# pouryashirazian/FemBrain

Measured on AMD Instinct MI355X. Metric: FEM steps/sec (assemble+PCG) at 1M tets, higher is better.
Workload: dtype f64 arithmetic / f32 stored matrix

## Files before the change

### fembrain_amd/csrc/fem_persist.hip

```cpp
#include <cmath>
#include <cstring>

#include "fem_handle.h"
#include "pcg_pipe.hip.h"
#include "pcg_pipe2.hip.h"
#include "pcg_pipe_plan.h"

using namespace fb;

namespace fb {

struct PipeKernel {
  int rows;
  bool c16;
  int wmax, klt;
  bool timing, shard, bj, help, xyz;
  const void* fn;
};

namespace {

#define FB_PIPE1(C16, WMAX, KLT, TIMING, SHARD, BJ, HELP, XYZ) \
  {1, C16, WMAX, KLT, TIMING, SHARD, BJ, HELP, XYZ, (const void*)k_pcg_pipe<float, C16, WMAX, KLT, TIMING, SHARD, BJ, HELP, XYZ>}
#define FB_PIPE2(C16, SHARD, XYZ) {2, C16, 12, kPipe2Klt, false, SHARD, false, false, XYZ, (const void*)k_pcg_pipe2<C16, SHARD, XYZ>}
// ... 193 lines not shown
  FB_TRY(pipe_layout(h, kn, &want_xyz));
  ps.pipe_xyz = ps.pipe_rows == 2 && want_xyz;
  if (ps.pipe_rows != 1 || !(want_h || want_xyz) || w > kPipeMaxWaves) return FB_OK;
  const PipeTasks T = pipe_help_tasks(P.slice_off.data(), P.n_slices, ps.pipe_wg_first_host.empty() ? nullptr : ps.pipe_wg_first_host.data(), nb, w, h->c16 != 0, want_h,
                                      want_xyz, kn);
  if (!(T.all > 0 || T.deepest > 6 || want_xyz || kn.helpers == 2)) return FB_OK;
  FB_TRY(ps.pipe_tasks.upload(T.tasks, h->stream));
  ps.pipe_wmax = 12;
  ps.pipe_slots_dealt = T.deepest;
  ps.pipe_help_waves = T.help_waves; ps.pipe_n_help = T.most; ps.pipe_help_tasks = T.all;
  ps.pipe_xyz = want_xyz;
  if (kn.verbose) fprintf(stderr, "[fembrain] persistent solver: %d helper tasks (at most %d per workgroup), widest slice %d slots, mean %.1f, up to %d slots of a slice in LDS; a slot's gathers touch %.1f lines in planes, %.1f node by node -> %s\n", T.all, T.most, mx, mean, T.deepest, ps.pipe_gather_lines[0], ps.pipe_gather_lines[1], want_xyz ? "node by node" : "planes");
  return FB_OK;
}

int alloc_persist(fb_fem_s* h, int nb, const PersistKnobs& kn) {
  const FemPlan& P = h->plan;
  PersistState& ps = h->ps;
  hipStream_t s = h->stream;
  ZeroBatch zb(s);
  FB_TRY(ps.pipe_post.alloc((size_t)2 * nb * 4));
  zb.add(ps.pipe_post);
  ps.pipe_flag_extra = P.n_ranks > 1 ? kP2PMaxRanks : 0;
  FB_TRY(ps.pipe_flags.alloc((size_t)nb + ps.pipe_flag_extra + 16));
  zb.add(ps.pipe_flags);
  const size_t n_pad = (size_t)P.n_slices * 64, nv = (size_t)3 * P.n_local + 2;
  FB_TRY(ps.pipe_planes.alloc(2 * 3 * n_pad));
  zb.add(ps.pipe_planes);
  FB_TRY(ps.pipe_z.alloc(nv));
  FB_TRY(ps.pipe_s.alloc(nv));
  FB_TRY(ps.pipe_state.alloc(2));
  zb.add(ps.pipe_state);
  if (kn.timing) {
    FB_TRY(ps.persist_timing.alloc((size_t)nb * kPipeMaxWaves * 6));
    FB_TRY(ps.persist_timing.zero(s));
  } else {
    ps.persist_timing.release();
  }
  static_assert(kPipeMaxBlocks <= 256, "k_slice_producers holds 256 workgroups in its 8 mask words");
  FB_TRY(ps.pipe_owner.alloc((size_t)std::max(1, P.n_slices)));
  FB_TRY(ps.pipe_mask.alloc((size_t)std::max(1, P.n_slices) * 8));
  FB_TRY(ps.pipe_prod.alloc((size_t)nb * kPipeMaxProducers));
  FB_TRY(ps.pipe_prod_count.alloc((size_t)nb));
  FB_TRY(ps.pipe_prod_xcd.alloc((size_t)nb));
  FB_TRY(ps.pipe_stats.alloc(2));
  zb.add(ps.pipe_stats);
  FB_TRY(zb.flush());
  hipLaunchKernelGGL(k_slice_owner, dim3(ceil_div(nb, kBlock)), dim3(kBlock), 0, s, P.n_slices, nb, ps.pipe_wg_first.p, ps.pipe_owner.p);
  hipLaunchKernelGGL(k_slice_producers, dim3(ceil_div(std::max(1, P.n_slices), kWavesPerBlock)), dim3(kBlock), 0, s, P.n_slices, P.n_owned, h->slice_off.p, h->colidx.p,
                     ps.pipe_owner.p, ps.pipe_mask.p);
  hipLaunchKernelGGL(k_wg_producers, dim3(ceil_div(nb, kBlock)), dim3(kBlock), 0, s, P.n_slices, nb, ps.pipe_wg_first.p, ps.pipe_mask.p, kn.poll_all ? 1 : 0, ps.pipe_prod.p, ps.pipe_prod_count.p,
                     ps.pipe_prod_xcd.p, ps.pipe_stats.p);
  FB_HIP(hipGetLastError());
  ps.pipe_stats_pending = true;
  ps.pipe_max_producers = 0;
  FB_TRY(ps.pipe_xcc.alloc((size_t)nb));
  zb.add(ps.pipe_xcc);
  return zb.flush();
}

}

bool auto_matrix_f64(const fb_fem_s* h, int n_nodes, int n_ranks) {
  const int cus = h->cu_limit > 0 ? std::min(h->cu_limit, h->n_cu_device) : h->n_cu_device;
  const int nb = std::min(kPipeMaxBlocks, (cus / 8) * 8);
  const int w = nb >= 8 ? ceil_div(ceil_div(ceil_div(n_nodes, 64), 8), nb / 8) : 0;
  const bool shard_persist_asked = n_ranks > 1 && read_persist_knobs().sharded;
// ... 135 lines not shown
  pa.timeout_ticks = ps.persist_timeout_ticks;
  pa.timing = ps.persist_timing.p;
  pa.planes = ps.pipe_planes.p; pa.n_pad = ps.shard_persist ? (size_t)ceil_div(h->plan.n_local, 64) * 64 : (size_t)h->plan.n_slices * 64;
  pa.pstate = ps.pipe_state.p;
  pa.tasks = ps.pipe_tasks.p; pa.n_help = ps.pipe_n_help;
  pa.wg_first = ps.pipe_wg_first.p;
  pa.mirror = ps.pipe_mir.p; pa.mir_addr = ps.pipe_mir_addr.p; pa.mir_wg = ps.pipe_mir_wg.p; pa.mir_pool = ps.pipe_mir_pool.p;
  const int cwaves = K.rows == 2 ? ceil_div(ps.persist_waves, 2) : ps.persist_waves;
  pa.service = cwaves + ps.pipe_help_waves < ps.pipe_wmax ? 1 : 0;
  pa.prefetch_slots = ps.persist_waves >= 9 ? (K.rows == 2 ? 3 : 4) : 0;
  ShardArgs sa;
  memset(&sa, 0, sizeof sa);
  if (ps.shard_persist) {
    sa.rank = h->plan.rank; sa.n_ranks = h->plan.n_ranks; sa.n_owned = h->plan.n_owned; sa.n_halo = h->plan.n_local - h->plan.n_owned;
    sa.box = ps.sbox; sa.peer_box = ps.sbox_peers.p; sa.peer_seg = ps.sh_peer_seg.p; sa.halo_cap = ps.sbox_halo_cap;
    sa.halo_off = ps.sh_halo_off.p; sa.row_send_off = ps.sh_row_send_off.p; sa.row_send_rank = ps.sh_row_send_rank.p; sa.row_send_pos = ps.sh_row_send_pos.p;
    sa.wg_send_mask = ps.sh_wg_send_mask.p; sa.n_senders = ps.sh_n_senders.p; sa.proxy_wg = ps.sh_proxy_wg.p; sa.n_proxy = ps.sh_n_proxy; sa.wg_duty = ps.sh_wg_duty.p; sa.wg_range = ps.sh_wg_range.p;
    sa.delay_ticks = remote_delay_ticks();
  }
  SellView sv = sell_view(h);
  const float *vals = (const float*)h->vals.p, *dlo = (const float*)h->dlo.p;
  const double* inv = K.bj ? h->invblk.p : h->invdiag.p;
  void* args[] = {&sv, &vals, &dlo, &inv, &b, &h->x.p, &h->r.p, &h->Ad.p, &ps.pipe_z.p, &ps.pipe_s.p, &h->d.p, &h->st.p, &pa, &sa};
  const size_t lds = 160 * 1024;
  const dim3 grid(ps.persist_blocks), block(64 * (cwaves + ps.pipe_help_waves + pa.service));
  FB_HIP(hipEventRecord(h->ev_p[0], h->stream));
  FB_HIP(hipFuncSetAttribute(K.fn, hipFuncAttributeMaxDynamicSharedMemorySize, (int)lds));
  FB_HIP(hipLaunchKernel(K.fn, grid, block, args, lds, h->stream));
  FB_HIP(hipEventRecord(h->ev_p[1], h->stream));
  return FB_OK;
}

void print_pipe_timing(fb_fem_s* h) {
  std::vector<long long> tm((size_t)h->ps.persist_blocks * kPipeMaxWaves * 6);
  if (h->ps.persist_timing.download(tm.data(), tm.size(), h->stream) != FB_OK) return;
  (void)h->ps.persist_timing.zero(h->stream);
  const char* names[5] = {"publish (drained)", "flag+wait+acquire", "product", "sums sweep", "recurrences(+refresh)"};
  for (int k = 0; k < 5; k++) {
    double mn = 1e30, mx = 0, av = 0;
    int cnt = 0;
    for (int b = 0; b < h->ps.persist_blocks; b++)
      for (int w = 0; w < h->ps.persist_waves; w++) {
        const long long* t = &tm[((size_t)b * kPipeMaxWaves + w) * 6];
        if (t[5] <= 0) continue;
        const double us = (double)t[k] / (double)t[5] * 0.01;
        mn = std::min(mn, us); mx = std::max(mx, us); av += us; cnt++;
      }
    fprintf(stderr, "[fembrain] pipelined PCG %-22s per iteration: avg %.2f us  min %.2f  max %.2f (over %d waves)\n", names[k], av / std::max(cnt, 1), mn, mx, cnt);
  }
  if (h->ps.pipe_timing_level >= 2) {
    for (int k = 1; k <= 2; k++) {
      fprintf(stderr, "[fembrain] %s by wavefront:", names[k]);
      for (int w = 0; w < h->ps.persist_waves; w++) {
        double av = 0; int cnt = 0;
        for (int b = 0; b < h->ps.persist_blocks; b++) { const long long* t = &tm[((size_t)b * kPipeMaxWaves + w) * 6]; if (t[5] > 0) { av += (double)t[k] / (double)t[5] * 0.01; cnt++; } }
        fprintf(stderr, " %.2f", av / std::max(cnt, 1));
      }
      fprintf(stderr, "\n[fembrain] %s by XCD (avg / max over its workgroups' slowest wavefront):", names[k]);
      for (int x = 0; x < 8; x++) {
        double av = 0, mx = 0; int cnt = 0;
        for (int b = x; b < h->ps.persist_blocks; b += 8) {
          double wmx = 0;
          for (int w = 0; w < h->ps.persist_waves; w++) { const long long* t = &tm[((size_t)b * kPipeMaxWaves + w) * 6]; if (t[5] > 0) wmx = std::max(wmx, (double)t[k] / (double)t[5] * 0.01); }
          av += wmx; mx = std::max(mx, wmx); cnt++;
        }
        fprintf(stderr, " %.2f/%.2f", av / std::max(cnt, 1), mx);
      }
      fprintf(stderr, "\n");
    }
    std::vector<std::pair<double, int>> slow;
    for (int b = 0; b < h->ps.persist_blocks; b++) {
      double wmx = 0;
      for (int w = 0; w < h->ps.persist_waves; w++) { const long long* t = &tm[((size_t)b * kPipeMaxWaves + w) * 6]; if (t[5] > 0) wmx = std::max(wmx, (double)t[2] / (double)t[5] * 0.01); }
      slow.push_back({wmx, b});
    }
    std::sort(slow.begin(), slow.end());
    fprintf(stderr, "[fembrain] slowest product of a workgroup: median %.2f us, fastest", slow[slow.size() / 2].first);
    for (int k = 0; k < 6 && k < (int)slow.size(); k++) fprintf(stderr, " wg%d %.2f", slow[k].second, slow[k].first);
    fprintf(stderr, "; slowest");
    for (int k = 0; k < 12 && k < (int)slow.size(); k++) fprintf(stderr, " wg%d %.2f", slow[slow.size() - 1 - k].second, slow[slow.size() - 1 - k].first);
    fprintf(stderr, "\n");
  }
}

}

extern "C" {

int fb_fem_sharded_persist(fb_fem_t h) {
  if (!h) return 0;
  return h->ps.shard_persist && h->ps.persist ? 1 : 0;
}

int fb_fem_set_sharded_persist(fb_fem_t h, int on) {
  CHECK_HANDLE(h);
  if (!h->ps.shard_persist || !h->ps.sbox) return fail(FB_EINVAL, "the sharded persistent solver is not attached to this handle (FEMBRAIN_SHARDED_PERSIST=1 at creation, <= %d slices per CU)", 2 * (kPipeMaxWaves - 1));
  if (on && h->ps.persist_broken) return fail(FB_EDEVICE, "the sharded persistent solver of this handle timed out before; it stays with the two-launch iteration");
  FB_HIP(hipStreamSynchronize(h->stream));
  h->ps.persist = on != 0;
  return FB_OK;
}

int fb_fem_persist_info(fb_fem_t h, int* waves_per_cu, int* workgroups, int* lds_slots) {
  if (!h) return fail(FB_EINVAL, "null FEM handle");
  if (waves_per_cu) *waves_per_cu = h->ps.persist ? h->ps.persist_waves : 0;
  if (workgroups) *workgroups = h->ps.persist ? h->ps.persist_blocks : 0;
// ... 91 lines not shown
```

### fembrain_amd/csrc/pcg_pipe.hip.h

```cpp
#pragma once
#include "fem_kernels.h"
#include "pcg_pipe_stream.hip.h"
#include "pcg_pipe_mirror.h"

namespace fb {

constexpr int kPipeMaxWaves = 12;
constexpr int kPipeMaxBlocks = 256;
constexpr int kPipeSyncDoubles = 2 * 16 + 2 * kPipeMaxBlocks + 8;
constexpr int kPipeMaxProducers = 64;
constexpr int pipe_slot_bytes(bool c16) { return c16 ? 9 * 256 + 128 : 10 * 256; }
constexpr int pipe_lds_slots(bool c16) { return c16 ? 65 : 62; }
static_assert(sizeof(double) * kPipeSyncDoubles + (size_t)pipe_lds_slots(false) * pipe_slot_bytes(false) <= 160 * 1024, "LDS budget of k_pcg_pipe");
static_assert(sizeof(double) * kPipeSyncDoubles + (size_t)pipe_lds_slots(true) * pipe_slot_bytes(true) <= 160 * 1024, "LDS budget of k_pcg_pipe<c16>");
static_assert(mir_slot_bytes(true) == pipe_slot_bytes(true) && mir_slot_bytes(false) == pipe_slot_bytes(false) && mir_lds_slots(true) == pipe_lds_slots(true) &&
              mir_lds_slots(false) == pipe_lds_slots(false) && kMirWaves == kPipeMaxWaves, "the LDS window's planner sees the kernel's LDS");
static_assert(pipe_lds_slots(true) * pipe_slot_bytes(true) / 4 < 65536 && pipe_lds_slots(false) * pipe_slot_bytes(false) / 4 < 65536, "16-bit LDS word addresses of the mirror layers");

struct PipeArgs {
  unsigned long long* post;
  unsigned int* flags;
  unsigned int* error;
  unsigned int* seqs;
  const int* producers;
  const int* prod_count;
  const int* prod_xcd;
  int plain_local;
  unsigned int* xcc;
  int prefetch_slots;
  int service;
  int start;
  int n_iters;
  double eps2;
  int max_iter;
  long long timeout_ticks;
  long long* timing;
  double* planes;
  size_t n_pad;
  double* pstate;
  const int* wg_first;
  const int4* tasks;
  int n_help;
  const int4* mirror;
  const unsigned short* mir_addr;
  const int2* mir_wg;
  const int* mir_pool;
};
constexpr int kPipeTaskStride = 16;
constexpr int kPipeMaxHelpers = 8;
constexpr int pipe_help_slots(bool c16) { return c16 ? 6 : 5; }
static_assert(pipe_help_slots(true) * pipe_slot_bytes(true) >= kPipeMaxHelpers * 3 * 64 * 8 && pipe_help_slots(false) * pipe_slot_bytes(false) >= kPipeMaxHelpers * 3 * 64 * 8, "helpers' hand-over area");

__device__ __forceinline__ void st_sc1_u64(unsigned long long* p, unsigned long long v) { __hip_atomic_store(p, v, __ATOMIC_RELAXED, __HIP_MEMORY_SCOPE_AGENT); }
__device__ __forceinline__ void st_sc1_u32(unsigned int* p, unsigned int v) { __hip_atomic_store(p, v, __ATOMIC_RELAXED, __HIP_MEMORY_SCOPE_AGENT); }
__device__ __forceinline__ unsigned int ld_sc1_u32(const unsigned int* p) { return __hip_atomic_load(p, __ATOMIC_RELAXED, __HIP_MEMORY_SCOPE_AGENT); }
__device__ __forceinline__ void st_sc1_f64(double* p, double v) { __hip_atomic_store(p, v, __ATOMIC_RELAXED, __HIP_MEMORY_SCOPE_AGENT); }
__device__ __forceinline__ void st_sc1_xyz(double* p, double x, double y, double z) {
  typedef double d2 __attribute__((ext_vector_type(2)));
  const d2 xy = {x, y};
  asm volatile("global_store_dwordx4 %0, %1, off sc1\n\tglobal_store_dwordx2 %0, %2, off offset:16 sc1" : : "v"(p), "v"(xy), "v"(z) : "memory");
}
__device__ __forceinline__ uint4 ld_sc1_u128(const void* p) {
  uint4 v;
  asm volatile("global_load_dwordx4 %0, %1, off sc1\n\ts_waitcnt vmcnt(0)" : "=v"(v) : "v"(p) : "memory");
  return v;
}

__device__ __forceinline__ double uniform_f64(double v) {
  const long long b = __double_as_longlong(v);
  const unsigned int lo = __builtin_amdgcn_readfirstlane((unsigned int)(b & 0xffffffffLL)), hi = __builtin_amdgcn_readfirstlane((unsigned int)((unsigned long long)b >> 32));
  return __longlong_as_double((long long)(((unsigned long long)hi << 32) | lo));
}
__device__ __forceinline__ bool uniform_flag(bool f) { return __builtin_amdgcn_readfirstlane(f ? 1 : 0) != 0; }

__host__ __device__ inline void pipe_slices(int n_slices, int n_blocks, int b, int* first, int* count) {
  const int xcd = b & 7, j = b >> 3, per = n_blocks >> 3;
  const int chunk = (n_slices + 7) >> 3;
  const int lo = xcd * chunk;
  int len = n_slices - lo;
  len = len < 0 ? 0 : (len > chunk ? chunk : len);
  const int base = len / per, rem = len - base * per;
// ... 316 lines not shown
      const int2 pw = pa.mir_wg[blockIdx.x];
      unsigned int* lmat = (unsigned int*)(lds + kPipeSyncDoubles);
      for (int e = threadIdx.x; e < pw.y; e += blockDim.x) {
        const MT* src = vals + pa.mir_pool[(size_t)blockIdx.x * kMirPoolMax + e];
        unsigned int* pe = lmat + pw.x + (e >> 6) * 9 * 64 + (e & 63);
#pragma unroll
        for (int j = 0; j < 9; j++) pe[(3 * (j % 3) + j / 3) * 64] = __float_as_uint((float)src[j * 64]);
      }
    }
  }
  double* ypart = (double*)((char*)(lds + kPipeSyncDoubles) + (size_t)(pipe_lds_slots(C16) - pipe_help_slots(C16)) * pipe_slot_bytes(C16));
  int own_k1 = width, help_sl = -1, hk0 = 0, hk1 = 0, help_idx = 0, help_so = 0;
  unsigned int help_mask = 0u;
  if constexpr (HELP) {
    const int4 tk = pa.tasks[(size_t)blockIdx.x * kPipeTaskStride + wv];
    const bool helper = !live && !spare && tk.x >= 0;
    own_k1 = __builtin_amdgcn_readfirstlane(live ? tk.z : width);
    help_mask = (unsigned int)__builtin_amdgcn_readfirstlane(live ? tk.w : 0);
    help_sl = __builtin_amdgcn_readfirstlane(helper ? first + tk.x : -1);
    hk0 = __builtin_amdgcn_readfirstlane(helper ? tk.y : 0); hk1 = __builtin_amdgcn_readfirstlane(helper ? tk.z : 0);
    help_idx = __builtin_amdgcn_readfirstlane(helper ? tk.w : 0);
    help_so = __builtin_amdgcn_readfirstlane(sv.slice_off[help_sl < 0 ? 0 : help_sl]);
  }
  const int n_prod = pa.prod_count[blockIdx.x];
  int my_prod = -1;
  if (wv == 0 && n_prod >= 0 && lane < n_prod) my_prod = pa.producers[(size_t)blockIdx.x * kPipeMaxProducers + lane];

  unsigned int send_mask = 0u;
  ShardBoxLayout BL = {};
  if constexpr (SHARD) { send_mask = sa.wg_send_mask[blockIdx.x]; BL = shard_box_layout(sa.halo_cap); }
  unsigned int pub = pa.seqs[0], sums = pa.seqs[1];
  const long long t_limit = pa.timeout_ticks;
  bool failed = false;
  long long tm[TIMING ? 6 : 1] = {0}, tprev = TIMING ? wall_clock64() : 0;
  auto lap = [&](int k) { if (TIMING) { const long long t = wall_clock64(); tm[k] += t - tprev; tprev = t; } };

  const bool plain_cand = !SHARD && pa.plain_local != 0 && pa.prod_xcd[blockIdx.x] == 0;
  bool through = true, xcc_known = false;
  unsigned int my_xcc = 0u;
  if constexpr (!SHARD) {
    asm volatile("s_getreg_b32 %0, hwreg(HW_REG_XCC_ID, 0, 4)" : "=s"(my_xcc));
    if (threadIdx.x == 0) st_sc1_u32(pa.xcc + blockIdx.x, ((pub + 1u) << 4) | my_xcc);
  }
  static_assert(!XYZ || HELP, "the node-by-node vector comes with the table-driven instantiation");
  const size_t xs = XYZ ? 1 : pa.n_pad, cs = XYZ ? 3 : 1;
  auto publish = [&](const double* vin) {
    pub++;
    double* pl = pa.planes + (size_t)(pub & 1u) * 3 * pa.n_pad;
    if (rvalid) {
      if (XYZ && through) {
        st_sc1_xyz(pl + 3 * (size_t)row, vin[0], vin[1], vin[2]);
      } else if (through) {
#pragma unroll
        for (int a = 0; a < 3; a++) st_sc1_f64(pl + a * xs + cs * (size_t)row, vin[a]);
      } else {
#pragma unroll
        for (int a = 0; a < 3; a++) pl[a * xs + cs * (size_t)row] = vin[a];
      }
      if constexpr (SHARD) shard_send_row(sa, BL, pub, send_beg, send_end, vin);
    }
  };
  auto product = [&](const double* vin, double* y, bool post_sums, bool late_acquire) {
    double* pl = pa.planes + (size_t)(pub & 1u) * 3 * pa.n_pad;
    asm volatile("s_waitcnt vmcnt(0)" ::: "memory");
    __syncthreads();
    lap(0);
    if (post_sums) sums++;
// ... 34 lines not shown
            if (b < nb) {
              const uint4 f = ld_sc1_u128(pa.flags + b);
              ok = (int)(f.x - pub) >= 0 && (b + 1 >= nb || (int)(f.y - pub) >= 0) && (b + 2 >= nb || (int)(f.z - pub) >= 0) && (b + 3 >= nb || (int)(f.w - pub) >= 0);
            }
            if (__ballot(!ok) == 0ULL) break;
            if (ld_sc1_u32(pa.error) != 0u || wall_clock64() - t0 > t_limit) { failed = true; break; }
            __builtin_amdgcn_s_sleep(1);
          }
        }
      }
      if (failed && lane == 0) st_sc1_u32(pa.error, 1u);
      if (late_acquire) __builtin_amdgcn_fence(__ATOMIC_ACQUIRE, "agent");
      if (plain_cand && !xcc_known && !failed) {
        const bool same = my_prod < 0 || ld_sc1_u32(pa.xcc + my_prod) == ((pub << 4) | my_xcc);
        const bool all_same = __ballot(!same) == 0ULL;
        if (lane == 0) bc[5] = all_same ? 1.0 : 0.0;
      }
      asm volatile("s_waitcnt vmcnt(0)" ::: "memory");
      if (lane == 0) bc[3] = (failed || ld_sc1_u32(pa.error) != 0u) ? 1.0 : 0.0;
    }
    __syncthreads();
    lap(1);
    if (uniform_flag(bc[3] != 0.0 || (SHARD && bc[4] != 0.0))) { failed = true; return; }
    if (plain_cand && !xcc_known) { through = !uniform_flag(bc[5] != 0.0); xcc_known = true; }
    double y0 = 0, y1 = 0, y2 = 0;
    if (rvalid) {
      MT u00 = m00, u01 = m01, u02 = m02, u11 = m11, u12 = m12, u22 = m22;
      asm volatile("" : "+v"(u00), "+v"(u01), "+v"(u02), "+v"(u11), "+v"(u12), "+v"(u22));
      const double l00 = (double)u00, l01 = (double)u01, l02 = (double)u02, l11 = (double)u11, l12 = (double)u12, l22 = (double)u22;
      y0 = l00 * vin[0] + l01 * vin[1] + l02 * vin[2];
      y1 = l01 * vin[0] + l11 * vin[1] + l12 * vin[2];
      y2 = l02 * vin[0] + l12 * vin[1] + l22 * vin[2];
    }
    if (live) {
      if constexpr (kMir) {
        if (mir_a > 0) {
          int so_k = so;
          asm volatile("" : "+s"(so_k));
          pipe_stream_slots<C16, XYZ>(mir_a, ((unsigned int)so_k * 9u * 64u + (unsigned int)lane) * (unsigned int)sizeof(float),
                                      ((unsigned int)so_k * 64u + (unsigned int)lane) * (unsigned int)(C16 ? sizeof(short) : sizeof(int)), vals,
                                      C16 ? (const void*)sv.coldelta : (const void*)sv.colidx, pl, pl + xs, pl + 2 * xs, row, y0, y1, y2);
        }
        const unsigned int* lmt = (const unsigned int*)((const char*)(lds + kPipeSyncDoubles) + mir_tab) + lane;
        const unsigned int* lmat = (const unsigned int*)(lds + kPipeSyncDoubles);
#pragma unroll
        for (int k = 0; k < kMirMax; k++) if (k < mir_m) {
          unsigned int addr, col;
          if constexpr (C16) { const unsigned int wd = lmt[k * 64]; addr = wd >> 16; col = (unsigned int)(row + (int)(short)(wd & 0xffffu)); }
          else { col = lmt[k * 96]; addr = ((const unsigned short*)(lmt - lane + k * 96 + 64))[lane]; }
          const unsigned int* pk = lmat + addr;
          const double* xp = pl + cs * (size_t)col;
          const double x0 = xp[0], x1 = xp[xs], x2 = xp[2 * xs];
          y0 += (double)__uint_as_float(pk[0 * 64]) * x0 + (double)__uint_as_float(pk[3 * 64]) * x1 + (double)__uint_as_float(pk[6 * 64]) * x2;
          y1 += (double)__uint_as_float(pk[1 * 64]) * x0 + (double)__uint_as_float(pk[4 * 64]) * x1 + (double)__uint_as_float(pk[7 * 64]) * x2;
          y2 += (double)__uint_as_float(pk[2 * 64]) * x0 + (double)__uint_as_float(pk[5 * 64]) * x1 + (double)__uint_as_float(pk[8 * 64]) * x2;
        }
      }
      if (sizeof(MT) == 4 && KLT >= 16) {
        double gx[KLT][3];
#pragma unroll
        for (int k = 0; k < KLT; k++) {
          const unsigned int col = k < KL ? lds_col(k) : 0u;
          const double* xp = pl + cs * (size_t)col;
          gx[k][0] = k < KL ? xp[0] : 0.0; gx[k][1] = k < KL ? xp[xs] : 0.0; gx[k][2] = k < KL ? xp[2 * xs] : 0.0;
        }
#pragma unroll
        for (int k = 0; k < KLT; k++) if (k < KL) {
          const unsigned int* lk = lres + (size_t)k * kValWords * 64;
          const double x0 = gx[k][0], x1 = gx[k][1], x2 = gx[k][2];
          y0 += (double)__uint_as_float(lk[0 * 64]) * x0 + (double)__uint_as_float(lk[1 * 64]) * x1 + (double)__uint_as_float(lk[2 * 64]) * x2;
          y1 += (double)__uint_as_float(lk[3 * 64]) * x0 + (double)__uint_as_float(lk[4 * 64]) * x1 + (double)__uint_as_float(lk[5 * 64]) * x2;
          y2 += (double)__uint_as_float(lk[6 * 64]) * x0 + (double)__uint_as_float(lk[7 * 64]) * x1 + (double)__uint_as_float(lk[8 * 64]) * x2;
        }
      } else if (sizeof(MT) == 4) {
#pragma unroll
        for (int k = 0; k < KLT; k++) if (k < KL) {
          const unsigned int* lk = lres + (size_t)k * kValWords * 64;
          const double* xp = pl + cs * (size_t)lds_col(k);
          const double x0 = xp[0], x1 = xp[xs], x2 = xp[2 * xs];
          y0 += (double)__uint_as_float(lk[0 * 64]) * x0 + (double)__uint_as_float(lk[1 * 64]) * x1 + (double)__uint_as_float(lk[2 * 64]) * x2;
          y1 += (double)__uint_as_float(lk[3 * 64]) * x0 + (double)__uint_as_float(lk[4 * 64]) * x1 + (double)__uint_as_float(lk[5 * 64]) * x2;
          y2 += (double)__uint_as_float(lk[6 * 64]) * x0 + (double)__uint_as_float(lk[7 * 64]) * x1 + (double)__uint_as_float(lk[8 * 64]) * x2;
        }
        if constexpr (HELP) {
          for (int kb = KLT; kb < KL; kb += KLT) {
            double gx[KLT][3];
#pragma unroll
            for (int j = 0; j < KLT; j++) {
              const int k = min(kb + j, KL - 1);
              const double* xp = pl + cs * (size_t)lds_col(k);
              gx[j][0] = xp[0]; gx[j][1] = xp[xs]; gx[j][2] = xp[2 * xs];
            }
#pragma unroll
            for (int j = 0; j < KLT; j++) if (kb + j < KL) {
              const unsigned int* lk = lres + (size_t)(kb + j) * kValWords * 64;
              const double x0 = gx[j][0], x1 = gx[j][1], x2 = gx[j][2];
              y0 += (double)__uint_as_float(lk[0 * 64]) * x0 + (double)__uint_as_float(lk[1 * 64]) * x1 + (double)__uint_as_float(lk[2 * 64]) * x2;
              y1 += (double)__uint_as_float(lk[3 * 64]) * x0 + (double)__uint_as_float(lk[4 * 64]) * x1 + (double)__uint_as_float(lk[5 * 64]) * x2;
              y2 += (double)__uint_as_float(lk[6 * 64]) * x0 + (double)__uint_as_float(lk[7 * 64]) * x1 + (double)__uint_as_float(lk[8 * 64]) * x2;
            }
          }
        }
      }
      const int n_str = own_k1 - k_after;
      if (n_str > 0) {
        int so_k = so + k_after;
        asm volatile("" : "+s"(so_k));
        pipe_stream_slots<C16, XYZ>(n_str, ((unsigned int)so_k * 9u * 64u + (unsigned int)lane) * (unsigned int)sizeof(float),
                               ((unsigned int)so_k * 64u + (unsigned int)lane) * (unsigned int)(C16 ? sizeof(short) : sizeof(int)), vals,
                               C16 ? (const void*)sv.coldelta : (const void*)sv.colidx, pl, pl + xs, pl + 2 * xs, row, y0, y1, y2);
      }
    }
    if constexpr (HELP) if (help_sl >= 0) {
      double h0 = 0, h1 = 0, h2 = 0;
      int so_k = help_so + hk0;
      asm volatile("" : "+s"(so_k));
      if (hk1 > hk0)
      pipe_stream_slots<C16, XYZ>(hk1 - hk0, ((unsigned int)so_k * 9u * 64u + (unsigned int)lane) * (unsigned int)sizeof(float),
                             ((unsigned int)so_k * 64u + (unsigned int)lane) * (unsigned int)(C16 ? sizeof(short) : sizeof(int)), vals,
                             C16 ? (const void*)sv.coldelta : (const void*)sv.colidx, pl, pl + xs, pl + 2 * xs, help_sl * 64 + lane, h0, h1, h2);
      double* hp = ypart + (size_t)help_idx * 3 * 64 + lane;
      hp[0] = h0; hp[64] = h1; hp[128] = h2;
    }
    y[0] = y0; y[1] = y1; y[2] = y2;
    lap(2);
  };
  auto add_helpers = [&](double* y) {
    unsigned int m = help_mask;
    while (m) {
      const int hi = __ffs((int)m) - 1;
      m &= m - 1u;
      const double* hp = ypart + (size_t)hi * 3 * 64 + lane;
      y[0] += hp[0]; y[1] += hp[64]; y[2] += hp[128];
    }
  };
// ... 153 lines not shown
#pragma unroll
    for (int a = 0; a < 3; a++) {
      zr[a] = y[a] + beta * zr[a];
      sr[a] = wr[a] + beta * sr[a];
    }
    if (!refresh) {
      double m[3];
#pragma unroll
      for (int a = 0; a < 3; a++) wr[a] = wr[a] - alpha * zr[a];
      precond(wr, m);
      publish(m);
      published = true;
    }
    if constexpr (BJ) {
      double ur[3];
      precond(rr, ur);
#pragma unroll
      for (int a = 0; a < 3; a++) pr[a] = ur[a] + beta * pr[a];
    } else {
#pragma unroll
      for (int a = 0; a < 3; a++) pr[a] = iv[a] * rr[a] + beta * pr[a];
    }
#pragma unroll
    for (int a = 0; a < 3; a++) xr[a] = xr[a] + alpha * pr[a];
    if (refresh) {
      phase = PH_REFRESH_X;
    } else {
#pragma unroll
      for (int a = 0; a < 3; a++) rr[a] = rr[a] - alpha * sr[a];
    }
    lap(4);
  }
  if (TIMING && lane == 0) {
    for (int k = 0; k < 5; k++) atomicAdd((unsigned long long*)pa.timing + ((size_t)blockIdx.x * kPipeMaxWaves + wv) * 6 + k, (unsigned long long)tm[k]);
    atomicAdd((unsigned long long*)pa.timing + ((size_t)blockIdx.x * kPipeMaxWaves + wv) * 6 + 5, (unsigned long long)it_done);
  }
  if (failed) return;
  const bool capped = done && gamma > eps2 * rho0;
  if (rvalid) {
    unsigned int dof = 3u * (unsigned int)row;
    asm volatile("" : "+v"(dof));
    if (capped) {
#pragma unroll
      for (int a = 0; a < 3; a++) pg[dof + a] = xr[a];
    } else {
#pragma unroll
      for (int a = 0; a < 3; a++) xg[dof + a] = xr[a];
      if (!done) {
#pragma unroll
        for (int a = 0; a < 3; a++) { rg[dof + a] = rr[a]; wg[dof + a] = wr[a]; zg[dof + a] = zr[a]; sg[dof + a] = sr[a]; pg[dof + a] = pr[a]; }
      }
    }
  }
  if (blockIdx.x == 0 && threadIdx.x == 0) {
    st->rho0 = rho0; st->eps2 = eps2; st->max_iter = max_iter;
    st->iter = iter;
    st->rho[iter & 1] = done ? gamma : gamma_old;
    st->done = done ? 1 : 0;
    pa.pstate[0] = gamma_old; pa.pstate[1] = alpha_old;
    pa.seqs[0] = (SHARD && published) ? pub - 1u : pub; pa.seqs[1] = sums;
  }
}

}
```

Baseline: 64.26.

## Software-pipeline on-chip mirrored and resident SpMV slots in hand-written assembly

Replaces the compiler-generated loop over LDS-mirrored slots, and the separate loop over LDS-resident plain slots, with one inline-assembly loop. It keeps up to four slot gathers of x in flight and uses graded vmcnt waits, so the gather latency overlaps with the f64 multiply-adds of earlier slots. It also adds timing seams that split the product phase into streamed and on-chip parts, with matching host-side reporting. The hand-written asm hardcodes VGPR numbers and LDS offsets, which adds register pressure and correctness risk.

```diff
diff --git a/fembrain_amd/csrc/fem_persist.hip b/fembrain_amd/csrc/fem_persist.hip
--- a/fembrain_amd/csrc/fem_persist.hip
+++ b/fembrain_amd/csrc/fem_persist.hip
@@ -249,7 +249,7 @@
   FB_TRY(ps.pipe_state.alloc(2));
   zb.add(ps.pipe_state);
   if (kn.timing) {
-    FB_TRY(ps.persist_timing.alloc((size_t)nb * kPipeMaxWaves * 6));
+    FB_TRY(ps.persist_timing.alloc((size_t)nb * kPipeMaxWaves * kPipeTimingSlots));
     FB_TRY(ps.persist_timing.zero(s));
   } else {
     ps.persist_timing.release();
@@ -451,7 +451,7 @@
 }
 
 void print_pipe_timing(fb_fem_s* h) {
-  std::vector<long long> tm((size_t)h->ps.persist_blocks * kPipeMaxWaves * 6);
+  std::vector<long long> tm((size_t)h->ps.persist_blocks * kPipeMaxWaves * kPipeTimingSlots);
   if (h->ps.persist_timing.download(tm.data(), tm.size(), h->stream) != FB_OK) return;
   (void)h->ps.persist_timing.zero(h->stream);
   const char* names[5] = {"publish (drained)", "flag+wait+acquire", "product", "sums sweep", "recurrences(+refresh)"};
@@ -460,19 +460,39 @@
     int cnt = 0;
     for (int b = 0; b < h->ps.persist_blocks; b++)
       for (int w = 0; w < h->ps.persist_waves; w++) {
-        const long long* t = &tm[((size_t)b * kPipeMaxWaves + w) * 6];
+        const long long* t = &tm[((size_t)b * kPipeMaxWaves + w) * kPipeTimingSlots];
         if (t[5] <= 0) continue;
         const double us = (double)t[k] / (double)t[5] * 0.01;
         mn = std::min(mn, us); mx = std::max(mx, us); av += us; cnt++;
       }
     fprintf(stderr, "[fembrain] pipelined PCG %-22s per iteration: avg %.2f us  min %.2f  max %.2f (over %d waves)\n", names[k], av / std::max(cnt, 1), mn, mx, cnt);
   }
+  if (h->ps.kernel && h->ps.kernel->wmax == 12 && !h->ps.kernel->help) {
+    const char* parts[3] = {"product: streamed [0,a)", "product: on-chip run", "product: streamed rest"};
+    for (int k = 0; k < 3; k++) {
+      double av = 0, mx = 0, sav = 0;
+      int cnt = 0, wgs = 0;
+      for (int b = 0; b < h->ps.persist_blocks; b++) {
+        double slowest = -1, part = 0;
+        for (int w = 0; w < h->ps.persist_waves; w++) {
+          const long long* t = &tm[((size_t)b * kPipeMaxWaves + w) * kPipeTimingSlots];
+          if (t[5] <= 0) continue;
+          const double us = (double)(k == 0 ? t[6] : (k == 1 ? t[7] : t[2] - t[6] - t[7])) / (double)t[5] * 0.01;
+          av += us; mx = std::max(mx, us); cnt++;
+          if ((double)t[2] > slowest) { slowest = (double)t[2]; part = us; }
+        }
+        if (slowest >= 0) { sav += part; wgs++; }
+      }
+      fprintf(stderr, "[fembrain] pipelined PCG %-24s per iteration: avg %.2f us  max %.2f; in the slowest wavefront of a workgroup: avg %.2f\n", parts[k], av / std::max(cnt, 1), mx,
+              sav / std::max(wgs, 1));
+    }
+  }
   if (h->ps.pipe_timing_level >= 2) {
     for (int k = 1; k <= 2; k++) {
       fprintf(stderr, "[fembrain] %s by wavefront:", names[k]);
       for (int w = 0; w < h->ps.persist_waves; w++) {
         double av = 0; int cnt = 0;
-        for (int b = 0; b < h->ps.persist_blocks; b++) { const long long* t = &tm[((size_t)b * kPipeMaxWaves + w) * 6]; if (t[5] > 0) { av += (double)t[k] / (double)t[5] * 0.01; cnt++; } }
+        for (int b = 0; b < h->ps.persist_blocks; b++) { const long long* t = &tm[((size_t)b * kPipeMaxWaves + w) * kPipeTimingSlots]; if (t[5] > 0) { av += (double)t[k] / (double)t[5] * 0.01; cnt++; } }
         fprintf(stderr, " %.2f", av / std::max(cnt, 1));
       }
       fprintf(stderr, "\n[fembrain] %s by XCD (avg / max over its workgroups' slowest wavefront):", names[k]);
@@ -480,7 +500,7 @@
         double av = 0, mx = 0; int cnt = 0;
         for (int b = x; b < h->ps.persist_blocks; b += 8) {
           double wmx = 0;
-          for (int w = 0; w < h->ps.persist_waves; w++) { const long long* t = &tm[((size_t)b * kPipeMaxWaves + w) * 6]; if (t[5] > 0) wmx = std::max(wmx, (double)t[k] / (double)t[5] * 0.01); }
+          for (int w = 0; w < h->ps.persist_waves; w++) { const long long* t = &tm[((size_t)b * kPipeMaxWaves + w) * kPipeTimingSlots]; if (t[5] > 0) wmx = std::max(wmx, (double)t[k] / (double)t[5] * 0.01); }
           av += wmx; mx = std::max(mx, wmx); cnt++;
         }
         fprintf(stderr, " %.2f/%.2f", av / std::max(cnt, 1), mx);
@@ -490,7 +510,7 @@
     std::vector<std::pair<double, int>> slow;
     for (int b = 0; b < h->ps.persist_blocks; b++) {
       double wmx = 0;
-      for (int w = 0; w < h->ps.persist_waves; w++) { const long long* t = &tm[((size_t)b * kPipeMaxWaves + w) * 6]; if (t[5] > 0) wmx = std::max(wmx, (double)t[2] / (double)t[5] * 0.01); }
+      for (int w = 0; w < h->ps.persist_waves; w++) { const long long* t = &tm[((size_t)b * kPipeMaxWaves + w) * kPipeTimingSlots]; if (t[5] > 0) wmx = std::max(wmx, (double)t[2] / (double)t[5] * 0.01); }
       slow.push_back({wmx, b});
     }
     std::sort(slow.begin(), slow.end());
diff --git a/fembrain_amd/csrc/pcg_pipe.hip.h b/fembrain_amd/csrc/pcg_pipe.hip.h
--- a/fembrain_amd/csrc/pcg_pipe.hip.h
+++ b/fembrain_amd/csrc/pcg_pipe.hip.h
@@ -1,6 +1,7 @@
 #pragma once
 #include "fem_kernels.h"
 #include "pcg_pipe_stream.hip.h"
+#include "pcg_pipe_onchip.hip.h"
 #include "pcg_pipe_mirror.h"
 
 namespace fb {
@@ -47,6 +48,7 @@
   const int* mir_pool;
 };
 constexpr int kPipeTaskStride = 16;
+constexpr int kPipeTimingSlots = 8;
 constexpr int kPipeMaxHelpers = 8;
 constexpr int pipe_help_slots(bool c16) { return c16 ? 6 : 5; }
 static_assert(pipe_help_slots(true) * pipe_slot_bytes(true) >= kPipeMaxHelpers * 3 * 64 * 8 && pipe_help_slots(false) * pipe_slot_bytes(false) >= kPipeMaxHelpers * 3 * 64 * 8, "helpers' hand-over area");
@@ -429,7 +431,8 @@
   unsigned int pub = pa.seqs[0], sums = pa.seqs[1];
   const long long t_limit = pa.timeout_ticks;
   bool failed = false;
-  long long tm[TIMING ? 6 : 1] = {0}, tprev = TIMING ? wall_clock64() : 0;
+  long long tm[TIMING ? 7 : 1] = {0}, tprev = TIMING ? wall_clock64() : 0;
+  auto seam = [&](int k, long long& t) { if (TIMING) { const long long u = wall_clock64(); tm[k] += u - t; t = u; } };
   auto lap = [&](int k) { if (TIMING) { const long long t = wall_clock64(); tm[k] += t - tprev; tprev = t; } };
 
   const bool plain_cand = !SHARD && pa.plain_local != 0 && pa.prod_xcd[blockIdx.x] == 0;
@@ -530,6 +533,7 @@
       y1 = l01 * vin[0] + l11 * vin[1] + l12 * vin[2];
       y2 = l02 * vin[0] + l12 * vin[1] + l22 * vin[2];
     }
+    long long tseam = tprev;
     if (live) {
       if constexpr (kMir) {
         if (mir_a > 0) {
@@ -539,20 +543,10 @@
                                       ((unsigned int)so_k * 64u + (unsigned int)lane) * (unsigned int)(C16 ? sizeof(short) : sizeof(int)), vals,
                                       C16 ? (const void*)sv.coldelta : (const void*)sv.colidx, pl, pl + xs, pl + 2 * xs, row, y0, y1, y2);
         }
-        const unsigned int* lmt = (const unsigned int*)((const char*)(lds + kPipeSyncDoubles) + mir_tab) + lane;
-        const unsigned int* lmat = (const unsigned int*)(lds + kPipeSyncDoubles);
-#pragma unroll
-        for (int k = 0; k < kMirMax; k++) if (k < mir_m) {
-          unsigned int addr, col;
-          if constexpr (C16) { const unsigned int wd = lmt[k * 64]; addr = wd >> 16; col = (unsigned int)(row + (int)(short)(wd & 0xffffu)); }
-          else { col = lmt[k * 96]; addr = ((const unsigned short*)(lmt - lane + k * 96 + 64))[lane]; }
-          const unsigned int* pk = lmat + addr;
-          const double* xp = pl + cs * (size_t)col;
-          const double x0 = xp[0], x1 = xp[xs], x2 = xp[2 * xs];
-          y0 += (double)__uint_as_float(pk[0 * 64]) * x0 + (double)__uint_as_float(pk[3 * 64]) * x1 + (double)__uint_as_float(pk[6 * 64]) * x2;
-          y1 += (double)__uint_as_float(pk[1 * 64]) * x0 + (double)__uint_as_float(pk[4 * 64]) * x1 + (double)__uint_as_float(pk[7 * 64]) * x2;
-          y2 += (double)__uint_as_float(pk[2 * 64]) * x0 + (double)__uint_as_float(pk[5 * 64]) * x1 + (double)__uint_as_float(pk[8 * 64]) * x2;
-        }
+        seam(5, tseam);
+        const char* lbase = (const char*)(lds + kPipeSyncDoubles);
+        pipe_onchip_slots<C16>(mir_m, max(KL, 0), (const unsigned int*)(lbase + mir_tab) + lane, (const unsigned short*)(lbase + mir_tab) + lane, lres, lcd, lbase, pl, pl + xs,
+                               pl + 2 * xs, row, y0, y1, y2);
       }
       if (sizeof(MT) == 4 && KLT >= 16) {
         double gx[KLT][3];
@@ -570,7 +564,7 @@
           y1 += (double)__uint_as_float(lk[3 * 64]) * x0 + (double)__uint_as_float(lk[4 * 64]) * x1 + (double)__uint_as_float(lk[5 * 64]) * x2;
           y2 += (double)__uint_as_float(lk[6 * 64]) * x0 + (double)__uint_as_float(lk[7 * 64]) * x1 + (double)__uint_as_float(lk[8 * 64]) * x2;
         }
-      } else if (sizeof(MT) == 4) {
+      } else if (sizeof(MT) == 4 && !kMir) {
 #pragma unroll
         for (int k = 0; k < KLT; k++) if (k < KL) {
           const unsigned int* lk = lres + (size_t)k * kValWords * 64;
@@ -599,6 +593,10 @@
             }
           }
         }
+      }
+      if constexpr (kMir) {
+        if (TIMING) asm volatile("" : "+v"(y0), "+v"(y1), "+v"(y2));
+        seam(6, tseam);
       }
       const int n_str = own_k1 - k_after;
       if (n_str > 0) {
@@ -818,8 +816,10 @@
     lap(4);
   }
   if (TIMING && lane == 0) {
-    for (int k = 0; k < 5; k++) atomicAdd((unsigned long long*)pa.timing + ((size_t)blockIdx.x * kPipeMaxWaves + wv) * 6 + k, (unsigned long long)tm[k]);
-    atomicAdd((unsigned long long*)pa.timing + ((size_t)blockIdx.x * kPipeMaxWaves + wv) * 6 + 5, (unsigned long long)it_done);
+    unsigned long long* tw = (unsigned long long*)pa.timing + ((size_t)blockIdx.x * kPipeMaxWaves + wv) * kPipeTimingSlots;
+    for (int k = 0; k < 5; k++) atomicAdd(tw + k, (unsigned long long)tm[k]);
+    atomicAdd(tw + 5, (unsigned long long)it_done);
+    atomicAdd(tw + 6, (unsigned long long)tm[5]); atomicAdd(tw + 7, (unsigned long long)tm[6]);
   }
   if (failed) return;
   const bool capped = done && gamma > eps2 * rho0;
diff --git a/fembrain_amd/csrc/pcg_pipe_onchip.hip.h b/fembrain_amd/csrc/pcg_pipe_onchip.hip.h
--- /dev/null
+++ b/fembrain_amd/csrc/pcg_pipe_onchip.hip.h
@@ -0,0 +1,171 @@
+#pragma once
+#include "pcg_pipe_stream.hip.h"
+
+namespace fb {
+
+#define FBO_ROW(y, x0, x1, x2, NEXT_AB, NEXT_C)                            \
+  "s_waitcnt lgkmcnt(0)\n\t"                                               \
+  "v_cvt_f64_f32_e32 v[120:121], v152\n\t"                                 \
+  "v_cvt_f64_f32_e32 v[122:123], v153\n\t"                                 \
+  NEXT_AB                                                                  \
+  "v_mul_f64 v[120:121], " x0 ", v[120:121]\n\t"                           \
+  "v_mul_f64 v[122:123], " x1 ", v[122:123]\n\t"                           \
+  "v_add_f64 v[120:121], v[120:121], v[122:123]\n\t"                       \
+  "v_cvt_f64_f32_e32 v[122:123], v154\n\t"                                 \
+  NEXT_C                                                                   \
+  "v_mul_f64 v[122:123], " x2 ", v[122:123]\n\t"                           \
+  "v_add_f64 v[120:121], v[120:121], v[122:123]\n\t"                       \
+  "v_add_f64 " y ", " y ", v[120:121]\n\t"
+#define FBO_READ_AB(A, o0, o1) "ds_read2st64_b32 v[152:153], " A " offset0:" o0 " offset1:" o1 "\n\t"
+#define FBO_READ_C(A, o2) "ds_read_b32 v154, " A " offset:" o2 "\n\t"
+#define FBO_COMPUTE_PLAIN(x0, x1, x2, A)                                                               \
+  FBO_ROW("%[y0]", x0, x1, x2, FBO_READ_AB(A, "3", "4"), FBO_READ_C(A, "1280"))                        \
+  FBO_ROW("%[y1]", x0, x1, x2, FBO_READ_AB(A, "6", "7"), FBO_READ_C(A, "2048"))                        \
+  FBO_ROW("%[y2]", x0, x1, x2, "", "")
+#define FBO_FIRST_PLAIN(A) FBO_READ_AB(A, "0", "1") FBO_READ_C(A, "512")
+#define FBO_COMPUTE_MIR(x0, x1, x2, A)                                                                 \
+  FBO_ROW("%[y0]", x0, x1, x2, FBO_READ_AB(A, "1", "4"), FBO_READ_C(A, "1792"))                        \
+  FBO_ROW("%[y1]", x0, x1, x2, FBO_READ_AB(A, "2", "5"), FBO_READ_C(A, "2048"))                        \
+  FBO_ROW("%[y2]", x0, x1, x2, "", "")
+#define FBO_FIRST_MIR(A) FBO_READ_AB(A, "0", "3") FBO_READ_C(A, "1536")
+#define FBO_GATHER(x0, x1, x2)                                             \
+  "global_load_dwordx2 " x0 ", v122, %[spl0]\n\t"                          \
+  "global_load_dwordx2 " x1 ", v122, %[spl1]\n\t"                          \
+  "global_load_dwordx2 " x2 ", v122, %[spl2]\n\t"
+#define FBO_ISSUE_MIR16(x0, x1, x2, A)                                     \
+  "ds_read_b32 " A ", %[lmt]\n\t"                                          \
+  "v_add_u32_e32 %[lmt], 0x100, %[lmt]\n\t"                                \
+  "s_waitcnt lgkmcnt(0)\n\t"                                               \
+  "v_bfe_i32 v122, " A ", 0, 16\n\t"                                       \
+  "v_add_u32_e32 v122, %[row], v122\n\t"                                   \
+  "v_lshlrev_b32_e32 v122, 3, v122\n\t"                                    \
+  FBO_GATHER(x0, x1, x2)                                                   \
+  "v_lshrrev_b32_e32 " A ", 16, " A "\n\t"                                 \
+  "v_lshl_add_u32 " A ", " A ", 2, %[lmat]\n\t"
+#define FBO_ISSUE_PLAIN16(x0, x1, x2, A)                                   \
+  "ds_read_i16 v122, %[lcd]\n\t"                                           \
+  "v_add_u32_e32 %[lcd], 0x80, %[lcd]\n\t"                                 \
+  "v_mov_b32_e32 " A ", %[lres]\n\t"                                       \
+  "v_add_u32_e32 %[lres], 0x900, %[lres]\n\t"                              \
+  "s_waitcnt lgkmcnt(0)\n\t"                                               \
+  "v_add_u32_e32 v122, %[row], v122\n\t"                                   \
+  "v_lshlrev_b32_e32 v122, 3, v122\n\t"                                    \
+  FBO_GATHER(x0, x1, x2)
+#define FBO_ISSUE_MIR32(x0, x1, x2, A)                                     \
+  "ds_read_b32 v122, %[lmt]\n\t"                                           \
+  "ds_read_u16 " A ", %[lmt2] offset:256\n\t"                              \
+  "v_add_u32_e32 %[lmt], 0x180, %[lmt]\n\t"                                \
+  "v_add_u32_e32 %[lmt2], 0x180, %[lmt2]\n\t"                              \
+  "s_waitcnt lgkmcnt(0)\n\t"                                               \
+  "v_lshlrev_b32_e32 v122, 3, v122\n\t"                                    \
+  FBO_GATHER(x0, x1, x2)                                                   \
+  "v_lshl_add_u32 " A ", " A ", 2, %[lmat]\n\t"
+#define FBO_ISSUE_PLAIN32(x0, x1, x2, A)                                   \
+  "ds_read_b32 v122, %[lres] offset:2304\n\t"                              \
+  "v_mov_b32_e32 " A ", %[lres]\n\t"                                       \
+  "v_add_u32_e32 %[lres], 0xa00, %[lres]\n\t"                              \
+  "s_waitcnt lgkmcnt(0)\n\t"                                               \
+  "v_lshlrev_b32_e32 v122, 3, v122\n\t"                                    \
+  FBO_GATHER(x0, x1, x2)
+#define FBO_ISSUE(J, ISSUE_MIR, ISSUE_PLAIN, x0, x1, x2, A)                \
+  "s_cmp_lt_i32 %[mi], 1\n\t"                                              \
+  "s_cbranch_scc1 .Lfbo_ip" J "_%=\n\t"                                    \
+  ISSUE_MIR(x0, x1, x2, A)                                                 \
+  "s_sub_i32 %[mi], %[mi], 1\n\t"                                          \
+  "s_add_i32 %[fl], %[fl], 1\n\t"                                          \
+  "s_branch .Lfbo_id" J "_%=\n"                                            \
+  ".Lfbo_ip" J "_%=:\n\t"                                                  \
+  "s_cmp_lt_i32 %[pi], 1\n\t"                                              \
+  "s_cbranch_scc1 .Lfbo_id" J "_%=\n\t"                                    \
+  ISSUE_PLAIN(x0, x1, x2, A)                                               \
+  "s_sub_i32 %[pi], %[pi], 1\n\t"                                          \
+  "s_add_i32 %[fl], %[fl], 1\n"                                            \
+  ".Lfbo_id" J "_%=:\n\t"
+#define FBO_WAITVM(J)                                                      \
+  "s_cmp_lt_i32 %[fl], 3\n\t"                                              \
+  "s_cbranch_scc1 .Lfbo_w2" J "_%=\n\t"                                    \
+  "s_waitcnt vmcnt(9)\n\t"                                                 \
+  "s_branch .Lfbo_wd" J "_%=\n"                                            \
+  ".Lfbo_w2" J "_%=:\n\t"                                                  \
+  "s_cmp_lt_i32 %[fl], 2\n\t"                                              \
+  "s_cbranch_scc1 .Lfbo_w1" J "_%=\n\t"                                    \
+  "s_waitcnt vmcnt(6)\n\t"                                                 \
+  "s_branch .Lfbo_wd" J "_%=\n"                                            \
+  ".Lfbo_w1" J "_%=:\n\t"                                                  \
+  "s_cmp_lt_i32 %[fl], 1\n\t"                                              \
+  "s_cbranch_scc1 .Lfbo_w0" J "_%=\n\t"                                    \
+  "s_waitcnt vmcnt(3)\n\t"                                                 \
+  "s_branch .Lfbo_wd" J "_%=\n"                                            \
+  ".Lfbo_w0" J "_%=:\n\t"                                                  \
+  "s_waitcnt vmcnt(0)\n"                                                   \
+  ".Lfbo_wd" J "_%=:\n\t"
+#define FBO_SLOT(J, ISSUE_MIR, ISSUE_PLAIN, x0, x1, x2, A)                 \
+  "s_cmp_lt_i32 %[nc], 1\n\t"                                              \
+  "s_cbranch_scc1 .Lfbo_end_%=\n\t"                                        \
+  "s_sub_i32 %[nc], %[nc], 1\n\t"                                          \
+  "s_sub_i32 %[fl], %[fl], 1\n\t"                                          \
+  "s_cmp_lt_i32 %[mc], 1\n\t"                                              \
+  "s_cbranch_scc1 .Lfbo_cp" J "_%=\n\t"                                    \
+  "s_sub_i32 %[mc], %[mc], 1\n\t"                                          \
+  FBO_FIRST_MIR(A)                                                         \
+  FBO_WAITVM("m" J)                                                        \
+  FBO_COMPUTE_MIR(x0, x1, x2, A)                                           \
+  "s_branch .Lfbo_ci" J "_%=\n"                                            \
+  ".Lfbo_cp" J "_%=:\n\t"                                                  \
+  FBO_FIRST_PLAIN(A)                                                       \
+  FBO_WAITVM("p" J)                                                        \
+  FBO_COMPUTE_PLAIN(x0, x1, x2, A)                                         \
+  ".Lfbo_ci" J "_%=:\n\t"                                                  \
+  FBO_ISSUE(J, ISSUE_MIR, ISSUE_PLAIN, x0, x1, x2, A)
+#define FBO_SET0 "v[124:125]", "v[126:127]", "v[128:129]", "v148"
+#define FBO_SET1 "v[130:131]", "v[132:133]", "v[134:135]", "v149"
+#define FBO_SET2 "v[136:137]", "v[138:139]", "v[140:141]", "v150"
+#define FBO_SET3 "v[142:143]", "v[144:145]", "v[146:147]", "v151"
+#define FBO_ISSUE_(J, ISSUE_MIR, ISSUE_PLAIN, SET) FBO_ISSUE(J, ISSUE_MIR, ISSUE_PLAIN, SET)
+#define FBO_SLOT_(J, ISSUE_MIR, ISSUE_PLAIN, SET) FBO_SLOT(J, ISSUE_MIR, ISSUE_PLAIN, SET)
+#define FBO_BODY(ISSUE_MIR, ISSUE_PLAIN)                                                                        \
+   \
+  "s_nop 4\n\t"                                                                                                 \
+  "s_mov_b32 %[fl], 0\n\t"                                                                                      \
+                                            \
+  FBO_ISSUE_("a", ISSUE_MIR, ISSUE_PLAIN, FBO_SET0)                                                             \
+  FBO_ISSUE_("b", ISSUE_MIR, ISSUE_PLAIN, FBO_SET1)                                                             \
+  FBO_ISSUE_("c", ISSUE_MIR, ISSUE_PLAIN, FBO_SET2)                                                             \
+  FBO_ISSUE_("d", ISSUE_MIR, ISSUE_PLAIN, FBO_SET3)                                                             \
+  ".Lfbo_loop_%=:\n\t"                                                                                          \
+  FBO_SLOT_("0", ISSUE_MIR, ISSUE_PLAIN, FBO_SET0)                                                              \
+  FBO_SLOT_("1", ISSUE_MIR, ISSUE_PLAIN, FBO_SET1)                                                              \
+  FBO_SLOT_("2", ISSUE_MIR, ISSUE_PLAIN, FBO_SET2)                                                              \
+  FBO_SLOT_("3", ISSUE_MIR, ISSUE_PLAIN, FBO_SET3)                                                              \
+  "s_branch .Lfbo_loop_%=\n"                                                                                    \
+  ".Lfbo_end_%=:\n\t"
+
+__device__ __forceinline__ unsigned int lds_byte_address(const void* p) {
+  return (unsigned int)(unsigned long long)(__attribute__((address_space(3))) const void*)p;
+}
+
+template <bool C16>
+__device__ __forceinline__ void pipe_onchip_slots(int m, int kl, const void* lmt, const void* lmt2, const void* lres, const void* lcd, const void* lmat,
+                                                  const double* pl0, const double* pl1, const double* pl2, int row, double& y0, double& y1, double& y2) {
+  pl0 = scalar_ptr(pl0); pl1 = scalar_ptr(pl1); pl2 = scalar_ptr(pl2);
+  int mi = __builtin_amdgcn_readfirstlane(m), pi = __builtin_amdgcn_readfirstlane(kl), mc = mi, nc = mi + pi, fl;
+  const unsigned int almat = __builtin_amdgcn_readfirstlane(lds_byte_address(lmat));
+  unsigned int almt = lds_byte_address(lmt), ares = lds_byte_address(lres);
+  if constexpr (C16) {
+    unsigned int acd = lds_byte_address(lcd);
+    asm volatile(FBO_BODY(FBO_ISSUE_MIR16, FBO_ISSUE_PLAIN16)
+                 : [y0] "+v"(y0), [y1] "+v"(y1), [y2] "+v"(y2), [lmt] "+v"(almt), [lres] "+v"(ares), [lcd] "+v"(acd), [mi] "+s"(mi), [pi] "+s"(pi),
+                   [mc] "+s"(mc), [nc] "+s"(nc), [fl] "=&s"(fl)
+                 : [lmat] "s"(almat), [spl0] "s"(pl0), [spl1] "s"(pl1), [spl2] "s"(pl2), [row] "v"(row)
+                 : FBP_CLOBBERS);
+  } else {
+    unsigned int almt2 = lds_byte_address(lmt2);
+    asm volatile(FBO_BODY(FBO_ISSUE_MIR32, FBO_ISSUE_PLAIN32)
+                 : [y0] "+v"(y0), [y1] "+v"(y1), [y2] "+v"(y2), [lmt] "+v"(almt), [lmt2] "+v"(almt2), [lres] "+v"(ares), [mi] "+s"(mi), [pi] "+s"(pi),
+                   [mc] "+s"(mc), [nc] "+s"(nc), [fl] "=&s"(fl)
+                 : [lmat] "s"(almat), [spl0] "s"(pl0), [spl1] "s"(pl1), [spl2] "s"(pl2)
+                 : FBP_CLOBBERS);
+  }
+}
+
+}
```

Result: faster. 67.86 (median of 6 runs) (+5.6%).
